# loxxous/Jampack

Hardware: AMD Instinct MI355X
Metric: MB/s compress (forward BWT + rANS encode) on 64 MiB blocks; bit-exact vs CPU ref (higher is better)
Workload: dtype u8/int32; 1 GPU; enwik8-like 100000000 B per GPU as 64 MiB blocks (2 blocks), forward BWT + rANS encode, inputs resident in HBM

## Files before the change

### jampack_amd/csrc/ans_enc.hip

```cpp
#include <vector>

#include "ans_enc.hpp"
#include "chain_pool.hpp"

using namespace jpk;
using namespace jpk_enc;

namespace {

void enc_layout(Arena &a, const EncDims &d, EncBufs &b, int what, size_t sym_total = 0, size_t lane_total = 0)
{
    const size_t tiles = (size_t)d.nch * d.tpc;
    const size_t stride = d.chunk;
    const size_t nsym = sym_total ? sym_total : (size_t)d.nch * stride;
    const size_t nlane = lane_total ? lane_total : (size_t)d.nch * 4 * rans_lane_stride(stride);
    const EncBufs keep = b;
    if (what & LAY_RANK) memset(&b, 0, sizeof b); else b = keep;
    if (what & LAY_RANK) {
        b.tilecnt = a.get<uint32_t>(tiles * 256);
        b.lastpos = a.get<int32_t>(tiles * 256);
        b.freq = a.get<int32_t>((size_t)d.nch * 256);
        b.bstart = a.get<uint32_t>((size_t)d.nch * 256);
        b.ranks = a.get<uint8_t>((size_t)d.nch * stride + 64);
    }
    if (what & LAY_RLE) {
        b.lz = a.get<uint32_t>(tiles);
        b.ext = a.get<uint32_t>(tiles);
        b.tcount = a.get<uint32_t>(tiles);
        b.toff = a.get<uint32_t>(tiles);
        b.rlen = a.get<uint32_t>(d.nch + 1);
        b.rle = a.get<uint16_t>((size_t)d.nch * stride + 64);
    }
    if (what & LAY_MODEL) {
        b.dens = a.get<uint32_t>(d.nch + 64);
        b.cmap = a.get<uint32_t>(d.nch + 64);
        b.clscnt = a.get<uint32_t>(tiles * 8);
        b.clstotal = a.get<uint32_t>((size_t)d.nch * 8);
        b.ord = a.get<uint32_t>(nsym);
        b.qhist = a.get<uint32_t>((size_t)d.nch * 6 * NQ * QSTRIDE);
        b.qcdf = a.get<uint32_t>((size_t)d.nch * 6 * NQ * QSTRIDE);
        b.exph = a.get<uint16_t>(7 * nsym);
        b.mantad = a.get<uint32_t>(nsym);
        b.cls8 = a.get<uint8_t>(nsym + 64);
        b.clist = a.get<uint32_t>(2 * ((nsym + 3) & ~(size_t)3) + 64);
        const size_t segs = (size_t)d.nch * 9 * d.tpc;
        b.seg_flag = a.get<uint32_t>(segs);
        b.seg_lo = a.get<int32_t>(segs);
        b.seg_end = a.get<int32_t>(segs);
        b.seg_start = a.get<int32_t>(segs);
        b.seg_tab = a.get<uint16_t>(segs * 32);
        b.seg_miss = a.get<uint16_t>(segs);
        b.seg_reach = a.get<uint16_t>(segs);
        b.recs = a.get<uint4>(nlane + RANS_SLACK) + (a.planning ? 0 : RANS_SLACK);
        b.pairs = (what & LAY_PLAIN) ? a.get<uint32_t>((size_t)d.nch * stride * 2) : nullptr;
    }
    if (what & LAY_RANS) {
        b.x16 = a.get<uint16_t>(nlane + 64);
        b.emask = a.get<uint32_t>(nlane / 16 + 64);
        b.etsum = a.get<uint32_t>((size_t)d.nch * emit_tiles_per_chunk(stride));
        b.fstate = a.get<uint32_t>((size_t)d.nch * 4);
        b.csize = a.get<uint32_t>(d.nch);
        b.stamp = a.get<uint64_t>(2 * (size_t)d.nch);
        b.hdr = a.get<uint8_t>((size_t)d.nch * HDR_MAX);
        b.hsize = a.get<uint32_t>(d.nch);
        b.outoff = a.get<uint64_t>(d.nch + 1);
    }
}

EncDims make_dims(uint32_t len, uint32_t chunk)
{
    EncDims d;
    d.len = len;
    d.chunk = chunk;
    d.nch = (len + chunk - 1) / chunk;
    d.tpc = (chunk + ATILE - 1) / ATILE;
    d.ncl = d.nch;
    d.cmap = nullptr;
    d.clen = nullptr;
    d.cblk = nullptr;
    d.bout = nullptr;
    d.sbase = nullptr;
    d.lbase = nullptr;
    return d;
}

__global__ __launch_bounds__(TB) void k_density(const uint8_t *__restrict__ in, EncDims d, uint32_t *__restrict__ dens)
{
    const uint32_t c = blockIdx.y, ts = blockIdx.x * ATILE * 4;
    const uint32_t clen = chunk_len(d, c);
    if (ts >= clen) return;
    const uint32_t te = (ts + ATILE * 4 < clen) ? ts + ATILE * 4 : clen;
    const uint8_t *src = in + (size_t)c * d.chunk;
    uint32_t n = 0;
    for (uint32_t i = ts + threadIdx.x * 16; i < te; i += TB * 16) {
        uint8_t prev = i ? src[i - 1] : 0;
        for (uint32_t k = 0; k < 16 && i + k < te; k++) { uint8_t v = src[i + k]; n += (v != prev); prev = v; }
    }
    n = wave_sum(n);
    if (lane_id() == 0 && n) atomicAdd(&dens[c], n);
}

__global__ __launch_bounds__(256) void k_order(EncDims d, const uint32_t *__restrict__ dens, uint32_t *__restrict__ cmap)
{
    for (uint32_t c = threadIdx.x; c < d.nch; c += blockDim.x) {
        const uint32_t v = dens[c];
        uint32_t r = 0;
        for (uint32_t k = 0; k < d.nch; k++) {
            const uint32_t w = dens[k];
            r += (w > v || (w == v && k < c)) ? 1u : 0u;
        }
        cmap[r] = c;
    }
}

constexpr uint32_t ENC_PLAN_SYM_256 = 141;

size_t enc_plan_bytes(const EncDims &d, int nblk, uint32_t sym_per_byte_256)
{
    EncBufs b;
    jpk_ctx dummy;
    Arena plan(&dummy, true);
    enc_layout(plan, d, b, LAY_RANK | LAY_RLE);
    plan.get<uint32_t>((size_t)d.nch + 1);
    plan.get<uint32_t>((size_t)d.nch + 1);
    if (nblk) { plan.get<uint32_t>(d.nch); plan.get<uint32_t>(d.nch); plan.get<uint8_t *>((size_t)nblk); }
    const size_t worst = (size_t)d.nch * d.chunk;
    size_t sym = worst / 256 * sym_per_byte_256 + 256 * (size_t)d.nch;
    if (sym > worst) sym = worst;
    enc_layout(plan, d, b, LAY_MODEL | LAY_RANS, sym, 2 * sym + 4 * 384 * (size_t)d.nch);
    return plan.need;
}

struct GroupTabs { const uint32_t *clen, *cblk; uint8_t *const *bout; int nblk; };

__global__ void k_sym_layout(EncDims d, const uint32_t *__restrict__ rlen, uint32_t *__restrict__ sbase, uint32_t *__restrict__ lbase, uint32_t *__restrict__ mail)
// ... 52 lines not shown

int enc_launch_groups(jpk_ctx *ctx, int inflight_n, uint32_t nch)
{
    int ngroups = jpk_enc_groups_for(inflight_n, nch);
    static const long groups_env = jpk_env_long("JPK_ENC_GROUPS", 0);
    if (groups_env >= 1 && groups_env <= jpk_ctx::ENC_GROUPS && (uint32_t)groups_env <= nch) ngroups = groups_env;
    for (int g = 0; g + 1 < ngroups; g++)
        if (!ctx->aux[g] && hipStreamCreateWithFlags(&ctx->aux[g], hipStreamNonBlocking) != hipSuccess) { ctx->aux[g] = nullptr; ngroups = g + 1; break; }
    return ngroups;
}

int enc_graded_groups(jpk_ctx *ctx, const uint8_t *d_in, const EncDims &d, EncBufs &b, int ngroups)
{
    hipStream_t st = ctx->stream;
    JPK_HIP(hipMemsetAsync(b.dens, 0, (size_t)d.nch * 4, st));
    JPK_LAUNCH(ctx, PROF_ENC_HIST, d.len, k_density, dim3((d.chunk + ATILE * 4 - 1) / (ATILE * 4), d.nch), dim3(TB), d_in, d, b.dens);
    JPK_LAUNCH(ctx, PROF_ENC_HIST, 0, k_order, dim3(1), dim3(256), d, b.dens, b.cmap);
    JPK_HIP(hipEventRecord(ctx->ev_pre[0], st));
    uint32_t gsz[jpk_ctx::ENC_GROUPS];
    {
        uint32_t left = d.nch;
        for (int g = 0; g < ngroups; g++) {
            uint32_t n = (g + 1 == ngroups) ? left : d.nch >> (ngroups - g);
            if (n < 2) n = 2;
            if (n > left) n = left;
            gsz[g] = n;
            left -= n;
        }
    }
    uint32_t off = 0;
    int rc = JPK_OK;
    for (int g = 0; g < ngroups && rc == JPK_OK; g++) {
        const uint32_t n = gsz[g];
        if (n == 0) continue;
        EncDims gd = d;
        gd.ncl = n; gd.cmap = b.cmap + off;
        off += n;
        hipStream_t gs = (g + 1 < ngroups) ? ctx->aux[g] : st;
        if (gs != st && hipStreamWaitEvent(gs, ctx->ev_pre[0], 0) != hipSuccess) { rc = JPK_E_DEVICE; break; }
        ctx->stream = gs;
        rc = run_model(ctx, b.rle, b.rlen, gd, b);
        if (rc == JPK_OK) rc = run_pairs(ctx, b.rle, b.rlen, gd, b);
        if (rc == JPK_OK) rc = run_chain(ctx, gd, b);
        if (rc == JPK_OK) rc = run_emit_counts(ctx, gd, b);
        ctx->stream = st;
        if (rc == JPK_OK && gs != st && hipEventRecord(ctx->ev_done[g], gs) != hipSuccess) rc = JPK_E_DEVICE;
    }
    for (int g = 0; g + 1 < ngroups && rc == JPK_OK; g++)
        if (hipStreamWaitEvent(st, ctx->ev_done[g], 0) != hipSuccess) rc = JPK_E_DEVICE;
    if (rc != JPK_OK) {
        for (int g = 0; g + 1 < jpk_ctx::ENC_GROUPS; g++) if (ctx->aux[g]) (void)hipStreamSynchronize(ctx->aux[g]);
        (void)hipStreamSynchronize(st);
    }
    return rc;
}

int enc_single_group(jpk_ctx *ctx, const EncDims &d, EncBufs &b)
{
    hipStream_t st = ctx->stream;
    JPK_TRY(run_model(ctx, b.rle, b.rlen, d, b));
    JPK_TRY(run_pairs(ctx, b.rle, b.rlen, d, b));
    JpkChainLease lease(ctx);
    if (lease.held()) {
        JPK_HIP(hipEventRecord(ctx->ev_pre[0], st));
        JPK_HIP(hipEventSynchronize(ctx->ev_pre[0]));
        ctx->stream = lease.stream;
        const int rc = run_chain(ctx, d, b);
        ctx->stream = st;
        JPK_TRY(rc);
        JPK_HIP(hipGetLastError());
        JPK_HIP(hipEventRecord(ctx->ev_done[0], lease.stream));
        JPK_HIP(hipEventSynchronize(ctx->ev_done[0]));
        lease.done();
    } else {
        JPK_TRY(run_chain(ctx, d, b));
    }
    JPK_TRY(run_emit_counts(ctx, d, b));
    return JPK_OK;
}

int encode_core(jpk_ctx *ctx, const uint8_t *d_in, EncDims &d, EncBufs &b, int inflight_n, const GroupTabs *gt = nullptr)
{
    JPK_TRY(enc_front(ctx, d_in, d, b, gt));
    JPK_HIP(hipMemsetAsync(b.qhist, 0, (size_t)d.nch * 6 * NQ * QSTRIDE * 4, ctx->stream));
    const int ngroups = enc_launch_groups(ctx, inflight_n, d.nch);
    if (ngroups >= 2) JPK_TRY(enc_graded_groups(ctx, d_in, d, b, ngroups));
    else JPK_TRY(enc_single_group(ctx, d, b));
    return run_offsets(ctx, d, b);
}
}

size_t jpk_ans_encode_arena_bytes(uint32_t len)
{
    if (len == 0) return 0;
    const EncDims d = make_dims(len, ANS_CHUNK);
    return enc_plan_bytes(d, 0, ENC_PLAN_SYM_256);
}
size_t jpk_ans_encode_arena_bytes_worst(uint32_t len)
{
    if (len == 0) return 0;
    const EncDims d = make_dims(len, ANS_CHUNK);
    return enc_plan_bytes(d, 0, 256);
}

int jpk_ans_encode_device(jpk_ctx *ctx, const uint8_t *d_in, int32_t len, uint8_t *d_out, int32_t out_cap, int32_t *out_len)
{
    const JpkCompressInflight inflight(ctx->device);
    *out_len = 0;
    ctx->stats.ans_chunks = 0;
    ctx->stats.ans_rle_symbols = 0;
    if (len == 0) return JPK_OK;
    hipStream_t st = ctx->stream;
    EncDims d = make_dims((uint32_t)len, ANS_CHUNK);
    EncBufs b;
    memset(&b, 0, sizeof b);
    JPK_TRY(encode_core(ctx, d_in, d, b, inflight.n));
    uint32_t mail[MAIL_OFFSETS_WORDS];
    JPK_TRY(jpk_read_mail(ctx, mail, MAIL_OFFSETS_WORDS));
    ctx->stats.enc_chain_cycles = (int64_t)mail_u64(mail, MAIL_CHAIN_CYCLES);
    ctx->stats.enc_chain_ns = (int64_t)mail_u64(mail, MAIL_CHAIN_TICKS) * 10;
    ctx->stats.enc_chain_steps = ((int64_t)mail[MAIL_CHAIN_RLEN] * 2 + 3) / 4;
    const uint64_t total = mail_u64(mail, MAIL_TOTAL);
    ctx->stats.ans_chunks = d.nch;
    ctx->stats.ans_rle_symbols = (int64_t)mail_u64(mail, MAIL_RLE_SYMBOLS);
    if (ctx->prof_on) {
        const uint64_t rs = (uint64_t)ctx->stats.ans_rle_symbols;
        ctx->prof_units[PROF_ENC_CLASS] += rs;
        ctx->prof_units[PROF_ENC_ADAPTIVE] += rs;
        ctx->prof_units[PROF_ENC_PAIRS] += rs;
        ctx->prof_units[PROF_ENC_RANS] += 2 * rs;
        ctx->prof_units[PROF_ENC_EMIT] += 2 * rs;
    }
    if (total > (uint64_t)out_cap) return JPK_E_CAPACITY;
    JPK_TRY(run_put(ctx, d, b, d_out));
    JPK_HIP(hipStreamSynchronize(st));
    *out_len = (int32_t)total;
    return JPK_OK;
}

size_t jpk_ans_encode_group_arena_bytes(uint32_t nchunks, int nblk)
{
    const EncDims d = make_dims(nchunks * ANS_CHUNK, ANS_CHUNK);
    return enc_plan_bytes(d, nblk, ENC_PLAN_SYM_256);
}

int jpk_ans_encode_group_device(jpk_ctx *ctx, int nblk, const uint8_t *d_stage, const uint32_t *first_chunk, const int32_t *mid_len, uint8_t *const *d_out,
                                const int32_t *out_cap, int32_t *out_len, int32_t *status)
{
    const JpkCompressInflight inflight(ctx->device);
    hipStream_t st = ctx->stream;
    std::vector<uint32_t> clen, cblk;
    for (int b = 0; b < nblk; b++) {
        out_len[b] = 0;
        status[b] = JPK_OK;
        const uint32_t ml = (uint32_t)mid_len[b], nc = (ml + ANS_CHUNK - 1) / ANS_CHUNK;
        if (clen.size() != first_chunk[b]) return JPK_E_ARG;
        for (uint32_t k = 0; k < nc; k++) {
            clen.push_back(k + 1 < nc ? (uint32_t)ANS_CHUNK : ml - k * (uint32_t)ANS_CHUNK);
            cblk.push_back((uint32_t)b);
        }
    }
    const uint32_t nch = (uint32_t)clen.size();
    if (nch == 0) return JPK_OK;
    EncDims d = make_dims(nch * ANS_CHUNK, ANS_CHUNK);
    EncBufs b;
    memset(&b, 0, sizeof b);
    const GroupTabs gt = {clen.data(), cblk.data(), d_out, nblk};
    JPK_TRY(encode_core(ctx, d_stage, d, b, inflight.n, &gt));
    uint8_t **d_bout = const_cast<uint8_t **>(d.bout);
    std::vector<uint32_t> hs(nch), cs(nch);
    JPK_HIP(hipMemcpyAsync(hs.data(), b.hsize, sizeof(uint32_t) * nch, hipMemcpyDeviceToHost, st));
    JPK_HIP(hipMemcpyAsync(cs.data(), b.csize, sizeof(uint32_t) * nch, hipMemcpyDeviceToHost, st));
    JPK_HIP(hipStreamSynchronize(st));
    std::vector<uint64_t> tot((size_t)nblk, 0);
    for (uint32_t c = 0; c < nch; c++) tot[cblk[c]] += (uint64_t)hs[c] + cs[c];
    bool all_fit = true;
    for (int k = 0; k < nblk; k++)
        if (tot[k] > (uint64_t)out_cap[k]) { status[k] = JPK_E_CAPACITY; all_fit = false; }
    if (!all_fit) {
        std::vector<uint8_t *> outs(d_out, d_out + nblk);
        for (int k = 0; k < nblk; k++) if (status[k] != JPK_OK) outs[k] = nullptr;
        JPK_HIP(hipMemcpyAsync(d_bout, outs.data(), sizeof(uint8_t *) * (size_t)nblk, hipMemcpyHostToDevice, st));
        JPK_HIP(hipStreamSynchronize(st));
    }
    JPK_TRY(run_put(ctx, d, b, nullptr));
    JPK_HIP(hipStreamSynchronize(st));
    for (int k = 0; k < nblk; k++) if (status[k] == JPK_OK) out_len[k] = (int32_t)tot[k];
    ctx->stats.ans_chunks = (int32_t)nch;
    return JPK_OK;
}

int jpk_rank_encode_device(jpk_ctx *ctx, uint8_t *d_t, int32_t *d_freq, int32_t len)
{
    if (len == 0) {
        JPK_HIP(hipMemsetAsync(d_freq, 0, 256 * 4, ctx->stream));
        return JPK_OK;
    }
    const EncDims d = make_dims((uint32_t)len, (uint32_t)len);
    EncBufs b;
    Arena plan(ctx, true);
    enc_layout(plan, d, b, LAY_RANK);
    JPK_TRY(jpk_arena_ensure(ctx, plan.need));
    Arena real(ctx, false);
    enc_layout(real, d, b, LAY_RANK);
    JPK_TRY(run_rank(ctx, d_t, d, b));
    JPK_HIP(hipMemcpyAsync(d_t, b.ranks, (size_t)len, hipMemcpyDeviceToDevice, ctx->stream));
    JPK_HIP(hipMemcpyAsync(d_freq, b.freq, 256 * 4, hipMemcpyDeviceToDevice, ctx->stream));
    return JPK_OK;
}

int jpk_rle_encode_device(jpk_ctx *ctx, const uint8_t *d_ranks, int32_t len, uint16_t *d_rle, int32_t *rlen)
{
    *rlen = 0;
    if (len == 0) return JPK_OK;
    const EncDims d = make_dims((uint32_t)len, (uint32_t)len);
    EncBufs b;
    Arena plan(ctx, true);
    enc_layout(plan, d, b, LAY_RLE);
    JPK_TRY(jpk_arena_ensure(ctx, plan.need));
    Arena real(ctx, false);
    enc_layout(real, d, b, LAY_RLE);
    JPK_TRY(run_rle(ctx, d_ranks, d, b));
    JPK_HIP(hipMemcpyAsync(ctx->d_mail->read, b.rlen, 4, hipMemcpyDeviceToDevice, ctx->stream));
    uint32_t n = 0;
    JPK_TRY(jpk_read_mail(ctx, &n, 1));
    JPK_HIP(hipMemcpyAsync(d_rle, b.rle, (size_t)n * 2, hipMemcpyDeviceToDevice, ctx->stream));
    JPK_HIP(hipStreamSynchronize(ctx->stream));
    *rlen = (int32_t)n;
    return JPK_OK;
}

int jpk_model_pairs_device(jpk_ctx *ctx, const uint16_t *d_rle, int32_t rlen, uint32_t *d_pairs)
{
    if (rlen == 0) return JPK_OK;
    const EncDims d = make_dims((uint32_t)rlen, (uint32_t)rlen);
    EncBufs b;
    Arena plan(ctx, true);
    enc_layout(plan, d, b, LAY_RLE | LAY_MODEL | LAY_PLAIN);
    JPK_TRY(jpk_arena_ensure(ctx, plan.need));
    Arena real(ctx, false);
    enc_layout(real, d, b, LAY_RLE | LAY_MODEL | LAY_PLAIN);
    uint32_t n = (uint32_t)rlen;
    JPK_HIP(hipMemcpyAsync(b.rlen, &n, 4, hipMemcpyHostToDevice, ctx->stream));
    JPK_HIP(hipStreamSynchronize(ctx->stream));
    JPK_HIP(hipMemsetAsync(b.qhist, 0, (size_t)d.nch * 6 * NQ * QSTRIDE * 4, ctx->stream));
    JPK_TRY(run_model(ctx, d_rle, b.rlen, d, b));
    JPK_TRY(run_pairs(ctx, d_rle, b.rlen, d, b));
    JPK_HIP(hipMemcpyAsync(d_pairs, b.pairs, (size_t)rlen * 8, hipMemcpyDeviceToDevice, ctx->stream));
    JPK_HIP(hipStreamSynchronize(ctx->stream));
    return JPK_OK;
}
```

### jampack_amd/csrc/ans_enc.hpp

```cpp
#pragma once
#include "ans_common.hpp"
#include "common.hpp"

namespace jpk_enc {
using namespace jpk;

constexpr int TB = 256;

struct EncDims {
    uint32_t len;
    uint32_t chunk;
    uint32_t nch;
    uint32_t tpc;
    uint32_t ncl;
    const uint32_t *cmap;
    const uint32_t *clen;
    const uint32_t *cblk;
    uint8_t *const *bout;
    const uint32_t *sbase;
    const uint32_t *lbase;
};
__device__ __forceinline__ uint32_t chunk_of(const EncDims &d, uint32_t i) { return d.cmap ? d.cmap[i] : i; }
__device__ __forceinline__ size_t sym_stride(const EncDims &d, uint32_t c, size_t rle_stride) { return d.sbase ? (size_t)(d.sbase[c + 1] - d.sbase[c]) : rle_stride; }
__device__ __forceinline__ size_t sym_base(const EncDims &d, uint32_t c, size_t rle_stride) { return d.sbase ? (size_t)d.sbase[c] : (size_t)c * rle_stride; }
__device__ __forceinline__ uint32_t chunk_len(const EncDims &d, uint32_t c)
{
    if (d.clen) return d.clen[c];
    uint64_t beg = (uint64_t)c * d.chunk;
    uint64_t left = d.len - beg;
    return left < d.chunk ? (uint32_t)left : d.chunk;
}

__host__ __device__ __forceinline__ size_t rans_lane_stride(size_t rle_stride) { return (rle_stride / 2 + 384) & ~(size_t)127; }
__device__ __forceinline__ size_t lane_stride_of(const EncDims &d, uint32_t c, size_t rle_stride) { return rans_lane_stride(sym_stride(d, c, rle_stride)); }
__device__ __forceinline__ size_t lane_base(const EncDims &d, uint32_t c, size_t rle_stride) { return d.lbase ? (size_t)d.lbase[c] : (size_t)c * 4 * rans_lane_stride(rle_stride); }

constexpr int RANS_RING = 16;
constexpr int RANS_SLACK = 16 * RANS_RING;
constexpr int ETILE = 4096;
constexpr int HDR_MAX = 259 * 5 + 1;
inline uint32_t emit_tiles_per_chunk(size_t stride) { return (uint32_t)((2 * stride + ETILE - 1) / ETILE); }

struct EncBufs {
    uint32_t *tilecnt; int32_t *lastpos; int32_t *freq; uint32_t *bstart; uint8_t *ranks;
    uint32_t *lz, *ext, *tcount, *toff, *rlen;
    uint16_t *rle;
    uint32_t *clscnt, *clstotal, *ord, *qhist, *qcdf, *dens, *cmap;
    uint8_t *cls8; uint32_t *clist;
    uint32_t *seg_flag; int32_t *seg_lo, *seg_end, *seg_start; uint16_t *seg_tab, *seg_miss, *seg_reach;
    uint16_t *exph; uint32_t *mantad, *pairs; uint4 *recs;
    uint16_t *x16; uint32_t *emask, *etsum, *fstate, *csize;
    uint64_t *stamp;
    uint8_t *hdr; uint32_t *hsize; uint64_t *outoff;
};

enum { LAY_RANK = 1, LAY_RLE = 2, LAY_MODEL = 4, LAY_RANS = 8, LAY_PLAIN = 16 };

constexpr int MAIL_TOTAL = 0;
constexpr int MAIL_RLE_SYMBOLS = 2;
constexpr int MAIL_CHAIN_CYCLES = 4;
constexpr int MAIL_CHAIN_TICKS = 6;
constexpr int MAIL_CHAIN_RLEN = 8;
constexpr int MAIL_SYM_TOTAL = 12;
constexpr int MAIL_LANE_TOTAL = 13;
constexpr int MAIL_OFFSETS_WORDS = 9, MAIL_LAYOUT_WORDS = 14;
static_assert(MAIL_LANE_TOTAL < JpkMail::READ_WORDS && MAIL_SYM_TOTAL < JpkMail::READ_WORDS, "the highest word lies inside JpkMail::read");
static_assert(MAIL_CHAIN_RLEN < MAIL_OFFSETS_WORDS && MAIL_CHAIN_TICKS + 1 < MAIL_OFFSETS_WORDS, "jpk_ans_encode_device's read covers k_out_offsets' words");
static_assert(MAIL_SYM_TOTAL < MAIL_LAYOUT_WORDS && MAIL_LANE_TOTAL < MAIL_LAYOUT_WORDS && MAIL_LAYOUT_WORDS <= JpkMail::READ_WORDS, "the front's read covers k_sym_layout's words");
static_assert(MAIL_SYM_TOTAL >= MAIL_OFFSETS_WORDS && MAIL_LANE_TOTAL >= MAIL_OFFSETS_WORDS && MAIL_SYM_TOTAL != MAIL_LANE_TOTAL, "k_sym_layout's words are none of k_out_offsets' nine");
static_assert(MAIL_TOTAL + 2 == MAIL_RLE_SYMBOLS && MAIL_RLE_SYMBOLS + 2 == MAIL_CHAIN_CYCLES && MAIL_CHAIN_CYCLES + 2 == MAIL_CHAIN_TICKS &&
              MAIL_CHAIN_TICKS + 2 == MAIL_CHAIN_RLEN, "four lo / hi pairs and one word, back to back");

int run_rank(jpk_ctx *ctx, const uint8_t *d_in, const EncDims &d, EncBufs &b);
int run_rle(jpk_ctx *ctx, const uint8_t *d_ranks, const EncDims &d, EncBufs &b);
int run_model(jpk_ctx *ctx, const uint16_t *d_rle, const uint32_t *d_rlen, const EncDims &d, EncBufs &b);
int run_pairs(jpk_ctx *ctx, const uint16_t *d_rle, const uint32_t *d_rlen, const EncDims &d, EncBufs &b);
int run_chain(jpk_ctx *ctx, const EncDims &d, EncBufs &b);
int run_emit_counts(jpk_ctx *ctx, const EncDims &d, EncBufs &b);
int run_offsets(jpk_ctx *ctx, const EncDims &d, EncBufs &b);
int run_put(jpk_ctx *ctx, const EncDims &d, EncBufs &b, uint8_t *d_out);

}
```

### jampack_amd/csrc/ans_enc_model.hip

```cpp
#include "ans_enc.hpp"

using namespace jpk;
using namespace jpk_enc;

namespace {

__global__ __launch_bounds__(TB) void k_cls_count(const uint16_t *__restrict__ rle, size_t rle_stride, EncDims d, const uint32_t *__restrict__ rlen,
                                                 uint32_t *__restrict__ clscnt)
{
    const uint32_t c = chunk_of(d, blockIdx.y), t = blockIdx.x;
    const uint32_t n = rlen[c], ts = t * ATILE;
    if (ts >= n) return;
    __shared__ uint32_t h[8];
    if (threadIdx.x < 8) h[threadIdx.x] = 0;
    __syncthreads();
    const uint16_t *src = rle + (size_t)c * rle_stride;
    uint32_t loc[8] = {0, 0, 0, 0, 0, 0, 0, 0};
    uint16_t sv[ATILE / TB];
#pragma unroll
    for (int it = 0; it < ATILE / TB; it++) {
        const uint32_t i = ts + it * TB + threadIdx.x;
        sv[it] = src[i < n ? i : n - 1];
    }
#pragma unroll
// ... 77 lines not shown
    }
    __syncthreads();
#pragma unroll
    for (int it = 0; it < IT; it++) {
        uint32_t i = ts + w * (64 * IT) + it * 64 + l;
        if (i < n) {
            uint32_t s = sy[it];
            int e = sym_class(s);
            uint32_t k = cnt[w][e] + rk[it];
            ord[sb + i] = k;
            cls8[sb + i] = (uint8_t)(e | ((s & 1u) << 3));
            if (e < 2) clist[2 * sb + (size_t)e * ((cs + 3) & ~(size_t)3) + k] = i | ((s & 1u) << 31);
            else {
                const int q = qinterval(k);
                const uint32_t m = s - (uint32_t)class_base(e);
                if (q == q0[e]) atomicAdd(&lh[e - 2][m], 1u);
                else atomicAdd(&qhist[(((size_t)c * 6 + (e - 2)) * NQ + q) * QSTRIDE + m], 1u);
            }
        }
    }
    __syncthreads();
    for (int i = threadIdx.x; i < 6 * QSTRIDE; i += TB) {
        const uint32_t v = (&lh[0][0])[i];
        if (v) {
            const int e2 = i / QSTRIDE, m = i % QSTRIDE;
            atomicAdd(&qhist[(((size_t)c * 6 + e2) * NQ + q0[e2 + 2]) * QSTRIDE + m], v);
        }
    }
}

__global__ __launch_bounds__(64) void k_quasi_build(EncDims d, const uint32_t *__restrict__ clstotal, const uint32_t *__restrict__ qhist,
                                                   uint32_t *__restrict__ qcdf)
{
    const int r = blockIdx.x, e = blockIdx.y + 2;
    const uint32_t c = chunk_of(d, blockIdx.z);
    const int A = class_alpha(e), l = lane_id();
    uint32_t *cdf = qcdf + (((size_t)c * 6 + (e - 2)) * NQ + r) * QSTRIDE;
    if (r == 0) {
        for (int i = l; i <= A; i += 64) cdf[i] = uniform_cdf(A, i);
        return;
    }
    if (clstotal[(size_t)c * 8 + e] < qbound(r)) return;
    const uint32_t *h = qhist + (((size_t)c * 6 + (e - 2)) * NQ + (r - 1)) * QSTRIDE;
    uint32_t F[3];
    uint32_t tot = 0;
#pragma unroll
    for (int k = 0; k < 3; k++) {
        int i = l + 64 * k;
        F[k] = (i < A) ? 16u * h[i] : 0u;
        tot += F[k];
    }
    tot = wave_sum(tot);
    int lg = 0;
    while ((tot >> lg) + (uint32_t)A > 65536u) lg++;
    uint32_t t2 = 0;
#pragma unroll
    for (int k = 0; k < 3; k++) {
        int i = l + 64 * k;
        F[k] = (i < A) ? (F[k] >> lg) + 1u : 0u;
        t2 += F[k];
    }
    t2 = wave_sum(t2);
    uint32_t t3 = 0;
#pragma unroll
    for (int k = 0; k < 3; k++) {
        F[k] = (65536u * F[k]) / t2;
        t3 += F[k];
    }
    t3 = wave_sum(t3);
    if (l == 0) F[0] += 65536u - t3;
    uint32_t carry = 0;
#pragma unroll
    for (int k = 0; k < 3; k++) {
        int i = l + 64 * k;
        uint32_t inc = wave_incl_sum(F[k]);
        if (i < A) cdf[i] = carry + inc - F[k];
        carry += __shfl(inc, 63, 64);
    }
    if (l == 0) cdf[A] = 65536u;
}

constexpr uint32_t AD_WARM_DEFAULT = 320;
static_assert(AD_WARM_DEFAULT % 64 == 0 && AD_WARM_DEFAULT >= 320 && AD_WARM_DEFAULT <= 4096, "whole waves of warm-up items, guarantee above");

struct AdRec {
    bool exp;
    int i;
    int cls;
    int A;
    __device__ __forceinline__ AdRec(uint32_t rec) : exp(rec < 7), i(rec < 7 ? (int)rec + 1 : 1), cls((int)rec - 7), A(rec < 7 ? 8 : 2) {}
    __device__ __forceinline__ int32_t init() const { return (int32_t)uniform_cdf(A, i); }
    __device__ __forceinline__ int32_t smin() const { return i; }
    __device__ __forceinline__ int32_t smax() const { return i + 65536 - A; }
};

__host__ __device__ __forceinline__ size_t clist_stride(size_t rle_stride) { return (rle_stride + 3) & ~(size_t)3; }

struct AdStream {
    const uint8_t *c8;
    const uint32_t *list;
    uint32_t n;
};
__device__ __forceinline__ AdStream ad_stream(const EncDims &d, const AdRec &r, uint32_t c, const uint8_t *cls8, const uint32_t *clist, size_t rle_stride,
                                              const uint32_t *rlen, const uint32_t *clstotal)
{
    AdStream st;
    const size_t sb = sym_base(d, c, rle_stride), cs = sym_stride(d, c, rle_stride);
    st.c8 = cls8 + sb;
    st.list = r.exp ? nullptr : clist + 2 * sb + (size_t)r.cls * clist_stride(cs);
    st.n = r.exp ? rlen[c] : clstotal[(size_t)c * 8 + r.cls];
    return st;
}

template <class F>
__device__ __forceinline__ void ad_for_each(const AdRec &r, const AdStream &st, uint32_t t0, uint32_t t1, F f)
{
    uint32_t t = t0;
    if (r.exp) {
        const uint8_t *p = st.c8;
        while (t < t1 && (t & 15u)) { f(t, (int)(p[t] & 7u)); t++; }
        if (t + 64 <= t1) {
            uint4 v[4];
#pragma unroll
            for (int q = 0; q < 4; q++) v[q] = *reinterpret_cast<const uint4 *>(p + t + 16 * q);
            for (; t + 64 <= t1; t += 64) {
                const uint32_t tn = (t + 128 <= t1) ? t + 64 : t;
                uint4 nv[4];
#pragma unroll
                for (int q = 0; q < 4; q++) nv[q] = *reinterpret_cast<const uint4 *>(p + tn + 16 * q);
#pragma unroll
                for (int q = 0; q < 4; q++) {
                    const uint32_t w[4] = {v[q].x, v[q].y, v[q].z, v[q].w};
#pragma unroll
                    for (int k = 0; k < 16; k++) f(t + 16 * q + k, (int)((w[k >> 2] >> (8 * (k & 3))) & 7u));
                }
#pragma unroll
                for (int q = 0; q < 4; q++) v[q] = nv[q];
            }
        }
        if (t + 16 <= t1) {
            uint4 v = *reinterpret_cast<const uint4 *>(p + t);
            for (; t + 16 <= t1; t += 16) {
                const uint32_t tn = (t + 32 <= t1) ? t + 16 : t;
                const uint4 nv = *reinterpret_cast<const uint4 *>(p + tn);
                const uint32_t w[4] = {v.x, v.y, v.z, v.w};
#pragma unroll
                for (int k = 0; k < 16; k++) f(t + k, (int)((w[k >> 2] >> (8 * (k & 3))) & 7u));
                v = nv;
            }
        }
        while (t < t1) { f(t, (int)(p[t] & 7u)); t++; }
    } else {
        const uint32_t *p = st.list;
        while (t < t1 && (t & 3u)) { const uint32_t e = p[t]; f(e & 0x7FFFFFFFu, (int)(e >> 31)); t++; }
        if (t + 16 <= t1) {
            uint4 v[4];
#pragma unroll
            for (int q = 0; q < 4; q++) v[q] = *reinterpret_cast<const uint4 *>(p + t + 4 * q);
            for (; t + 16 <= t1; t += 16) {
                const uint32_t tn = (t + 32 <= t1) ? t + 16 : t;
                uint4 nv[4];
#pragma unroll
                for (int q = 0; q < 4; q++) nv[q] = *reinterpret_cast<const uint4 *>(p + tn + 4 * q);
#pragma unroll
                for (int q = 0; q < 4; q++) {
                    f(v[q].x & 0x7FFFFFFFu, (int)(v[q].x >> 31));
// ... 13 lines not shown
                f(v.x & 0x7FFFFFFFu, (int)(v.x >> 31));
                f(v.y & 0x7FFFFFFFu, (int)(v.y >> 31));
                f(v.z & 0x7FFFFFFFu, (int)(v.z >> 31));
                f(v.w & 0x7FFFFFFFu, (int)(v.w >> 31));
                v = nv;
            }
        }
        while (t < t1) { const uint32_t e = p[t]; f(e & 0x7FFFFFFFu, (int)(e >> 31)); t++; }
    }
}

__device__ __forceinline__ int32_t ad_run_write(const AdRec &r, const AdStream &st, uint32_t t0, uint32_t t1, int32_t x,
                                                uint16_t *__restrict__ hist, uint32_t *__restrict__ ma)
{
    if (r.exp) {
        const int i = r.i;
        const uint8_t *p = st.c8;
        uint32_t t = t0;
        while (t < t1 && (t & 15u)) { hist[t] = (uint16_t)x; x = adapt_step(x, i, (int)(p[t] & 7u), 8); t++; }
        if (t + 64 <= t1) {
            uint4 v[4];
#pragma unroll
            for (int q = 0; q < 4; q++) v[q] = *reinterpret_cast<const uint4 *>(p + t + 16 * q);
            for (; t + 64 <= t1; t += 64) {
                const uint32_t tn = (t + 128 <= t1) ? t + 64 : t;
                uint4 nv[4];
#pragma unroll
                for (int q = 0; q < 4; q++) nv[q] = *reinterpret_cast<const uint4 *>(p + tn + 16 * q);
#pragma unroll
                for (int q = 0; q < 4; q++) {
                    const uint32_t w[4] = {v[q].x, v[q].y, v[q].z, v[q].w};
                    uint32_t o[8];
#pragma unroll
                    for (int k = 0; k < 16; k++) {
                        if (k & 1) o[k >> 1] |= (uint32_t)x << 16;
                        else o[k >> 1] = (uint32_t)x & 0xffffu;
                        x = adapt_step(x, i, (int)((w[k >> 2] >> (8 * (k & 3))) & 7u), 8);
                    }
                    uint4 *qq = reinterpret_cast<uint4 *>(hist + t + 16 * q);
                    qq[0] = make_uint4(o[0], o[1], o[2], o[3]);
                    qq[1] = make_uint4(o[4], o[5], o[6], o[7]);
                }
#pragma unroll
                for (int q = 0; q < 4; q++) v[q] = nv[q];
            }
        }
        if (t + 16 <= t1) {
            uint4 v = *reinterpret_cast<const uint4 *>(p + t);
            for (; t + 16 <= t1; t += 16) {
                const uint32_t tn = (t + 32 <= t1) ? t + 16 : t;
                const uint4 nv = *reinterpret_cast<const uint4 *>(p + tn);
                const uint32_t w[4] = {v.x, v.y, v.z, v.w};
                uint32_t o[8];
#pragma unroll
                for (int k = 0; k < 16; k++) {
                    if (k & 1) o[k >> 1] |= (uint32_t)x << 16;
                    else o[k >> 1] = (uint32_t)x & 0xffffu;
                    x = adapt_step(x, i, (int)((w[k >> 2] >> (8 * (k & 3))) & 7u), 8);
                }
                uint4 *q = reinterpret_cast<uint4 *>(hist + t);
                q[0] = make_uint4(o[0], o[1], o[2], o[3]);
                q[1] = make_uint4(o[4], o[5], o[6], o[7]);
                v = nv;
            }
        }
        while (t < t1) { hist[t] = (uint16_t)x; x = adapt_step(x, i, (int)(p[t] & 7u), 8); t++; }
    } else {
        ad_for_each(r, st, t0, t1, [&](uint32_t t, int m) {
            const uint32_t l0 = m ? (uint32_t)x : 0u, fr = m ? 65536u - (uint32_t)x : (uint32_t)x;
            ma[t] = l0 | (fr << 16);
            x = adapt_step(x, 1, m, 2);
        });
    }
    return x;
}

struct AdArgs {
    const uint8_t *cls8; const uint32_t *clist; size_t rle_stride; const uint32_t *rlen; const uint32_t *clstotal;
    const uint32_t *clsbase;
    uint16_t *exph; uint32_t *mantad;
    uint32_t warm;
    uint32_t *seg_flag; int32_t *seg_lo, *seg_end, *seg_start; uint16_t *seg_tab;
    uint16_t *seg_miss, *seg_reach;
};

__global__ __launch_bounds__(64) void k_adapt_a(EncDims d, AdArgs a)
{
    const uint32_t c = chunk_of(d, blockIdx.z), rec = blockIdx.y;
    const uint32_t k = blockIdx.x * 64 + threadIdx.x;
    const AdRec r(rec);
    const AdStream st = ad_stream(d, r, c, a.cls8, a.clist, a.rle_stride, a.rlen, a.clstotal);
    const uint32_t nt = (st.n + ATILE - 1) / ATILE;
    const bool valid = k < nt;
    const uint32_t t0 = valid ? k * ATILE : 0u, t1 = !valid ? 0u : (t0 + ATILE < st.n) ? t0 + ATILE : st.n;
    const uint32_t len = t1 - t0;
    const int i = r.i, A = r.A;
    int32_t lo = r.init(), hi = lo;
    if (valid && k != 0) {
        lo = r.smin(); hi = r.smax();
        ad_for_each(r, st, t0 - a.warm, t0, [&](uint32_t, int sy) { lo = adapt_step(lo, i, sy, A); hi = adapt_step(hi, i, sy, A); });
    }
    const size_t so = ((size_t)c * 9 + rec) * d.tpc + k;
    const int32_t lo0 = lo, hi0 = hi;
    const bool plat = valid && r.exp && lo != hi && hi == r.smax() && lo == r.smax() - 31;
    bool ident = false;
    if (plat) {
        const uint32_t *cb = a.clsbase + ((size_t)c * d.tpc + k) * 8;
        uint32_t reach = 0;
        for (int e = r.i; e < 8; e++) reach += ((k + 1 < nt) ? cb[8 + e] : a.clstotal[(size_t)c * 8 + e]) - cb[e];
        ident = reach == 0;
    }
    const bool walk = valid && !ident;
    bool open = walk && lo != hi, quiet = plat;
    uint32_t miss = 0, fr = 0, u = 0;
    uint16_t *hist = a.exph + 7 * sym_base(d, c, a.rle_stride) + (size_t)(rec < 7 ? rec : 0) * sym_stride(d, c, a.rle_stride);
    uint32_t *ma = a.mantad + sym_base(d, c, a.rle_stride);
    if (r.exp) {
        const uint8_t *p = st.c8 + t0;
        const int32_t top = r.smax();
        uint4 v[4];
        if (__ballot(open && 64u <= len)) {
#pragma unroll
            for (int q = 0; q < 4; q++) v[q] = *reinterpret_cast<const uint4 *>(p + ((walk && 64u <= len) ? 16 * q : 0));
        }
        while (__ballot(open && u + 64 <= len)) {
            const bool in = walk && u + 64 <= len;
            const uint32_t un = (in && u + 128 <= len) ? u + 64 : (in ? u : 0u);
            uint4 nv[4];
#pragma unroll
            for (int q = 0; q < 4; q++) nv[q] = *reinterpret_cast<const uint4 *>(p + un + 16 * q);
            if (in) {
#pragma unroll
                for (int q = 0; q < 4; q++) {
                    const uint32_t w[4] = {v[q].x, v[q].y, v[q].z, v[q].w};
                    const bool one = lo == hi;
                    uint32_t o[8];
#pragma unroll
                    for (int j = 0; j < 16; j++) {
                        if (j & 1) o[j >> 1] |= (uint32_t)lo << 16;
                        else o[j >> 1] = (uint32_t)lo & 0xffffu;
                        const int sy = (int)((w[j >> 2] >> (8 * (j & 3))) & 7u);
                        lo = adapt_step(lo, i, sy, 8);
                        hi = adapt_step(hi, i, sy, 8);
                    }
                    if (one) {
                        uint4 *qq = reinterpret_cast<uint4 *>(hist + t0 + u + 16 * q);
                        qq[0] = make_uint4(o[0], o[1], o[2], o[3]);
                        qq[1] = make_uint4(o[4], o[5], o[6], o[7]);
                    }
                    if (quiet) { if (hi == top) fr = u + 16 * q + 16; else quiet = false; }
                    if (open && lo == hi) { open = false; miss = u + 16 * q + 16; }
                }
            }
#pragma unroll
            for (int q = 0; q < 4; q++) v[q] = nv[q];
            u += 64;
        }
        if (walk && u > (len & ~63u)) u = len & ~63u;
    } else {
        const uint32_t *p = st.list + t0;
        uint4 v[4];
        if (__ballot(open && 16u <= len)) {
#pragma unroll
            for (int q = 0; q < 4; q++) v[q] = *reinterpret_cast<const uint4 *>(p + ((walk && 16u <= len) ? 4 * q : 0));
        }
        while (__ballot(open && u + 16 <= len)) {
            const bool in = walk && u + 16 <= len;
            const uint32_t un = (in && u + 32 <= len) ? u + 16 : (in ? u : 0u);
            uint4 nv[4];
#pragma unroll
            for (int q = 0; q < 4; q++) nv[q] = *reinterpret_cast<const uint4 *>(p + un + 4 * q);
            if (in) {
                const bool one = lo == hi;
#pragma unroll
                for (int q = 0; q < 4; q++) {
                    const uint32_t w[4] = {v[q].x, v[q].y, v[q].z, v[q].w};
#pragma unroll
                    for (int j = 0; j < 4; j++) {
                        const int m = (int)(w[j] >> 31);
                        if (one) {
                            const uint32_t l0 = m ? (uint32_t)lo : 0u, f = m ? 65536u - (uint32_t)lo : (uint32_t)lo;
                            ma[w[j] & 0x7FFFFFFFu] = l0 | (f << 16);
                        }
                        lo = adapt_step(lo, 1, m, 2);
                        hi = adapt_step(hi, 1, m, 2);
                    }
                }
                if (open && lo == hi) { open = false; miss = u + 16; }
            }
#pragma unroll
            for (int q = 0; q < 4; q++) v[q] = nv[q];
            u += 16;
        }
        if (walk && u > (len & ~15u)) u = len & ~15u;
    }
    if (!valid) return;
    if (ident) {
        a.seg_flag[so] = 2u;
        return;
    }
    if (open) {
        ad_for_each(r, st, t0 + u, t1, [&](uint32_t, int sy) { lo = adapt_step(lo, i, sy, A); hi = adapt_step(hi, i, sy, A); });
        a.seg_miss[so] = (uint16_t)len;
        a.seg_reach[so] = (uint16_t)fr;
        if (lo == hi) { a.seg_flag[so] = 3u; a.seg_end[so] = lo; }
        else { a.seg_flag[so] = 0u; a.seg_lo[so] = lo0; a.seg_end[so] = hi0; }
        return;
    }
    a.seg_flag[so] = miss ? 3u : 1u;
    a.seg_miss[so] = (uint16_t)miss;
    a.seg_reach[so] = (uint16_t)fr;
    a.seg_end[so] = ad_run_write(r, st, t0 + u, t1, lo, hist, ma);
}

__global__ __launch_bounds__(64) void k_adapt_tab(EncDims d, AdArgs a)
{
    const uint32_t c = chunk_of(d, blockIdx.z), rec = blockIdx.y;
    const uint32_t k = blockIdx.x * 2 + (threadIdx.x >> 5);
    const int q = threadIdx.x & 31;
    const AdRec r(rec);
    const AdStream st = ad_stream(d, r, c, a.cls8, a.clist, a.rle_stride, a.rlen, a.clstotal);
    const uint32_t nt = (st.n + ATILE - 1) / ATILE;
    if (k >= nt) return;
    const size_t so = ((size_t)c * 9 + rec) * d.tpc + k;
    if (a.seg_flag[so]) return;
    const uint32_t t0 = k * ATILE, t1 = (t0 + ATILE < st.n) ? t0 + ATILE : st.n;
    const int32_t lo = a.seg_lo[so], hi = a.seg_end[so];
    int32_t x = (lo + q < hi) ? lo + q : hi;
    const int i = r.i, A = r.A;
    ad_for_each(r, st, t0, t1, [&](uint32_t, int sy) { x = adapt_step(x, i, sy, A); });
    a.seg_tab[so * 32 + q] = (uint16_t)(x - 1);
}

__global__ __launch_bounds__(64) void k_adapt_b(EncDims d, AdArgs a)
{
    const uint32_t g = blockIdx.x * 64 + threadIdx.x;
    const uint32_t rec = g & 15u;
    if ((g >> 4) >= d.ncl || rec >= 9) return;
    const uint32_t c = chunk_of(d, g >> 4);
    const AdRec r(rec);
    const AdStream st = ad_stream(d, r, c, a.cls8, a.clist, a.rle_stride, a.rlen, a.clstotal);
    const uint32_t nt = (st.n + ATILE - 1) / ATILE;
    int32_t x = r.init();
    for (uint32_t k = 0; k < nt; k++) {
        const size_t so = ((size_t)c * 9 + rec) * d.tpc + k;
        const uint32_t flag = a.seg_flag[so];
        if (flag == 1u) x = a.seg_end[so];
        else if (flag == 2u) a.seg_start[so] = x;
        else if (flag == 3u) { a.seg_start[so] = x; x = a.seg_end[so]; }
        else {
            a.seg_start[so] = x;
            int q = x - a.seg_lo[so];
            q = q < 0 ? 0 : (q > 31 ? 31 : q);
            x = (int32_t)a.seg_tab[so * 32 + q] + 1;
        }
    }
}

__global__ __launch_bounds__(64) void k_adapt_c(EncDims d, AdArgs a)
{
    const uint32_t c = chunk_of(d, blockIdx.z), rec = blockIdx.y;
    const uint32_t k = blockIdx.x * 64 + threadIdx.x;
    const AdRec r(rec);
    const AdStream st = ad_stream(d, r, c, a.cls8, a.clist, a.rle_stride, a.rlen, a.clstotal);
    const uint32_t nt = (st.n + ATILE - 1) / ATILE;
    if (k >= nt) return;
    const size_t so = ((size_t)c * 9 + rec) * d.tpc + k;
    const uint32_t flag = a.seg_flag[so];
    if (flag == 1u) return;
    const uint32_t t0 = k * ATILE, t1 = (t0 + ATILE < st.n) ? t0 + ATILE : st.n;
    const uint32_t miss = flag == 2u ? t1 - t0 : a.seg_miss[so], fr = flag == 2u ? t1 - t0 : a.seg_reach[so];
    uint16_t *hist = a.exph + 7 * sym_base(d, c, a.rle_stride) + (size_t)(rec < 7 ? rec : 0) * sym_stride(d, c, a.rle_stride);
    const int32_t x0 = a.seg_start[so];
    if (fr) {
        const uint32_t x = (uint32_t)x0 & 0xffffu, xx = x | (x << 16);
        uint32_t t = t0;
        for (; t + 8 <= t0 + fr; t += 8) *reinterpret_cast<uint4 *>(hist + t) = make_uint4(xx, xx, xx, xx);
        for (; t < t0 + fr; t++) hist[t] = (uint16_t)x;
    }
    if (fr < miss) ad_run_write(r, st, t0 + fr, t0 + miss, x0, hist, a.mantad + sym_base(d, c, a.rle_stride));
}

}

namespace jpk_enc {

int run_model(jpk_ctx *ctx, const uint16_t *d_rle, const uint32_t *d_rlen, const EncDims &d, EncBufs &b)
{
    const size_t stride = d.chunk;
    JPK_LAUNCH(ctx, PROF_ENC_CLASS, 0, k_cls_count, dim3(d.tpc, d.ncl), dim3(TB), d_rle, stride, d, d_rlen, b.clscnt);
    JPK_LAUNCH(ctx, PROF_ENC_CLASS, 0, k_cls_prefix, dim3(jpk_grid((size_t)d.ncl * 8, 64)), dim3(64), d, d_rlen, b.clscnt, b.clstotal);
    JPK_LAUNCH(ctx, PROF_ENC_CLASS, 0, k_cls_ord, dim3(d.tpc, d.ncl), dim3(TB), d_rle, stride, d, d_rlen, b.clscnt, b.ord, b.qhist, b.cls8, b.clist);
    JPK_LAUNCH(ctx, PROF_ENC_CLASS, 0, k_quasi_build, dim3(NQ, 6, d.ncl), dim3(64), d, b.clstotal, b.qhist, b.qcdf);
    AdArgs aa;
    aa.cls8 = b.cls8; aa.clist = b.clist; aa.rle_stride = stride; aa.rlen = d_rlen; aa.clstotal = b.clstotal; aa.clsbase = b.clscnt;
    aa.exph = b.exph; aa.mantad = b.mantad;
    aa.warm = AD_WARM_DEFAULT;
    aa.seg_flag = b.seg_flag; aa.seg_lo = b.seg_lo; aa.seg_end = b.seg_end; aa.seg_start = b.seg_start; aa.seg_tab = b.seg_tab;
    aa.seg_miss = b.seg_miss; aa.seg_reach = b.seg_reach;
    JPK_LAUNCH(ctx, PROF_ENC_ADAPTIVE, 0, k_adapt_a, dim3((d.tpc + 63) / 64, 9, d.ncl), dim3(64), d, aa);
    JPK_LAUNCH(ctx, PROF_ENC_ADAPTIVE, 0, k_adapt_tab, dim3((d.tpc + 1) / 2, 9, d.ncl), dim3(64), d, aa);
    JPK_LAUNCH(ctx, PROF_ENC_ADAPTIVE, 0, k_adapt_b, dim3(jpk_grid((size_t)d.ncl * 16, 64)), dim3(64), d, aa);
    JPK_LAUNCH(ctx, PROF_ENC_ADAPTIVE, 0, k_adapt_c, dim3((d.tpc + 63) / 64, 9, d.ncl), dim3(64), d, aa);
    JPK_HIP(hipGetLastError());
    return JPK_OK;
}

}
```

Before: 6344 MB/s.

## Split adaptive-model segments into sub-tiles with compacted table worklist and wave scan

Adaptive-model segments shrink from a full tile to AD_SUB-sized sub-tiles, so the per-segment walk in k_adapt_a/k_adapt_c exposes more parallelism. Segments that need a 32-entry transfer table are compacted into a worklist via an atomic counter, so k_adapt_tab runs a fixed grid over only real work instead of a dense grid. k_adapt_b replaces a serial per-thread chain walk with a wave-level ballot/shuffle scan over 64 segments at a time. The cost is more segment metadata, a repeated warm-up per sub-tile, an atomic counter per chunk, and a counter word appended to the zeroed qhist region.

```diff
diff --git a/jampack_amd/csrc/ans_enc.hip b/jampack_amd/csrc/ans_enc.hip
--- a/jampack_amd/csrc/ans_enc.hip
+++ b/jampack_amd/csrc/ans_enc.hip
@@ -37,13 +37,14 @@
         b.clscnt = a.get<uint32_t>(tiles * 8);
         b.clstotal = a.get<uint32_t>((size_t)d.nch * 8);
         b.ord = a.get<uint32_t>(nsym);
-        b.qhist = a.get<uint32_t>((size_t)d.nch * 6 * NQ * QSTRIDE);
+        b.qhist = a.get<uint32_t>(model_zero_words(d.nch));
+        b.seg_nwork = a.planning ? nullptr : b.qhist + (size_t)d.nch * 6 * NQ * QSTRIDE;
         b.qcdf = a.get<uint32_t>((size_t)d.nch * 6 * NQ * QSTRIDE);
         b.exph = a.get<uint16_t>(7 * nsym);
         b.mantad = a.get<uint32_t>(nsym);
         b.cls8 = a.get<uint8_t>(nsym + 64);
         b.clist = a.get<uint32_t>(2 * ((nsym + 3) & ~(size_t)3) + 64);
-        const size_t segs = (size_t)d.nch * 9 * d.tpc;
+        const size_t segs = (size_t)d.nch * 9 * d.tpc * AD_PER_TILE;
         b.seg_flag = a.get<uint32_t>(segs);
         b.seg_lo = a.get<int32_t>(segs);
         b.seg_end = a.get<int32_t>(segs);
@@ -51,6 +52,7 @@
         b.seg_tab = a.get<uint16_t>(segs * 32);
         b.seg_miss = a.get<uint16_t>(segs);
         b.seg_reach = a.get<uint16_t>(segs);
+        b.seg_work = a.get<uint32_t>(segs);
         b.recs = a.get<uint4>(nlane + RANS_SLACK) + (a.planning ? 0 : RANS_SLACK);
         b.pairs = (what & LAY_PLAIN) ? a.get<uint32_t>((size_t)d.nch * stride * 2) : nullptr;
     }
@@ -269,7 +271,7 @@
 int encode_core(jpk_ctx *ctx, const uint8_t *d_in, EncDims &d, EncBufs &b, int inflight_n, const GroupTabs *gt = nullptr)
 {
     JPK_TRY(enc_front(ctx, d_in, d, b, gt));
-    JPK_HIP(hipMemsetAsync(b.qhist, 0, (size_t)d.nch * 6 * NQ * QSTRIDE * 4, ctx->stream));
+    JPK_HIP(hipMemsetAsync(b.qhist, 0, model_zero_words(d.nch) * 4, ctx->stream));
     const int ngroups = enc_launch_groups(ctx, inflight_n, d.nch);
     if (ngroups >= 2) JPK_TRY(enc_graded_groups(ctx, d_in, d, b, ngroups));
     else JPK_TRY(enc_single_group(ctx, d, b));
@@ -430,7 +432,7 @@
     uint32_t n = (uint32_t)rlen;
     JPK_HIP(hipMemcpyAsync(b.rlen, &n, 4, hipMemcpyHostToDevice, ctx->stream));
     JPK_HIP(hipStreamSynchronize(ctx->stream));
-    JPK_HIP(hipMemsetAsync(b.qhist, 0, (size_t)d.nch * 6 * NQ * QSTRIDE * 4, ctx->stream));
+    JPK_HIP(hipMemsetAsync(b.qhist, 0, model_zero_words(d.nch) * 4, ctx->stream));
     JPK_TRY(run_model(ctx, d_rle, b.rlen, d, b));
     JPK_TRY(run_pairs(ctx, d_rle, b.rlen, d, b));
     JPK_HIP(hipMemcpyAsync(d_pairs, b.pairs, (size_t)rlen * 8, hipMemcpyDeviceToDevice, ctx->stream));
diff --git a/jampack_amd/csrc/ans_enc.hpp b/jampack_amd/csrc/ans_enc.hpp
--- a/jampack_amd/csrc/ans_enc.hpp
+++ b/jampack_amd/csrc/ans_enc.hpp
@@ -41,6 +41,14 @@
 constexpr int HDR_MAX = 259 * 5 + 1;
 inline uint32_t emit_tiles_per_chunk(size_t stride) { return (uint32_t)((2 * stride + ETILE - 1) / ETILE); }
 
+#ifndef JPK_AD_SUB
+#define JPK_AD_SUB 1024
+#endif
+constexpr int AD_SUB = JPK_AD_SUB;
+constexpr int AD_PER_TILE = ATILE / AD_SUB;
+static_assert(AD_SUB >= 512 && AD_SUB <= ATILE && (AD_SUB & (AD_SUB - 1)) == 0 && ATILE % AD_SUB == 0, "a power of two that divides the tile, longer than a warm-up");
+inline size_t model_zero_words(uint32_t nch) { return (size_t)nch * 6 * NQ * QSTRIDE + nch; }
+
 struct EncBufs {
     uint32_t *tilecnt; int32_t *lastpos; int32_t *freq; uint32_t *bstart; uint8_t *ranks;
     uint32_t *lz, *ext, *tcount, *toff, *rlen;
@@ -48,6 +56,7 @@
     uint32_t *clscnt, *clstotal, *ord, *qhist, *qcdf, *dens, *cmap;
     uint8_t *cls8; uint32_t *clist;
     uint32_t *seg_flag; int32_t *seg_lo, *seg_end, *seg_start; uint16_t *seg_tab, *seg_miss, *seg_reach;
+    uint32_t *seg_work, *seg_nwork;
     uint16_t *exph; uint32_t *mantad, *pairs; uint4 *recs;
     uint16_t *x16; uint32_t *emask, *etsum, *fstate, *csize;
     uint64_t *stamp;
diff --git a/jampack_amd/csrc/ans_enc_model.hip b/jampack_amd/csrc/ans_enc_model.hip
--- a/jampack_amd/csrc/ans_enc_model.hip
+++ b/jampack_amd/csrc/ans_enc_model.hip
@@ -183,6 +183,7 @@
 
 constexpr uint32_t AD_WARM_DEFAULT = 320;
 static_assert(AD_WARM_DEFAULT % 64 == 0 && AD_WARM_DEFAULT >= 320 && AD_WARM_DEFAULT <= 4096, "whole waves of warm-up items, guarantee above");
+static_assert(AD_WARM_DEFAULT <= (uint32_t)AD_SUB && AD_SUB % 64 == 0, "a warm-up starts inside the stream; whole 64-item groups, 16-byte stores");
 
 struct AdRec {
     bool exp;
@@ -362,7 +363,10 @@
     uint32_t warm;
     uint32_t *seg_flag; int32_t *seg_lo, *seg_end, *seg_start; uint16_t *seg_tab;
     uint16_t *seg_miss, *seg_reach;
+    uint32_t *work, *nwork;
+    uint32_t spc;
 };
+__device__ __forceinline__ uint32_t ad_subs(const AdStream &st) { return (st.n + AD_SUB - 1) / AD_SUB; }
 
 __global__ __launch_bounds__(64) void k_adapt_a(EncDims d, AdArgs a)
 {
@@ -370,9 +374,10 @@
     const uint32_t k = blockIdx.x * 64 + threadIdx.x;
     const AdRec r(rec);
     const AdStream st = ad_stream(d, r, c, a.cls8, a.clist, a.rle_stride, a.rlen, a.clstotal);
-    const uint32_t nt = (st.n + ATILE - 1) / ATILE;
-    const bool valid = k < nt;
-    const uint32_t t0 = valid ? k * ATILE : 0u, t1 = !valid ? 0u : (t0 + ATILE < st.n) ? t0 + ATILE : st.n;
+    const uint32_t ns = ad_subs(st);
+    if (blockIdx.x * 64 >= ns) return;
+    const bool valid = k < ns;
+    const uint32_t t0 = valid ? k * AD_SUB : 0u, t1 = !valid ? 0u : (t0 + AD_SUB < st.n) ? t0 + AD_SUB : st.n;
     const uint32_t len = t1 - t0;
     const int i = r.i, A = r.A;
     int32_t lo = r.init(), hi = lo;
@@ -380,14 +385,15 @@
         lo = r.smin(); hi = r.smax();
         ad_for_each(r, st, t0 - a.warm, t0, [&](uint32_t, int sy) { lo = adapt_step(lo, i, sy, A); hi = adapt_step(hi, i, sy, A); });
     }
-    const size_t so = ((size_t)c * 9 + rec) * d.tpc + k;
+    const size_t so = ((size_t)c * 9 + rec) * a.spc + k;
     const int32_t lo0 = lo, hi0 = hi;
     const bool plat = valid && r.exp && lo != hi && hi == r.smax() && lo == r.smax() - 31;
     bool ident = false;
     if (plat) {
-        const uint32_t *cb = a.clsbase + ((size_t)c * d.tpc + k) * 8;
+        const uint32_t tile = k / AD_PER_TILE, nt = (st.n + ATILE - 1) / ATILE;
+        const uint32_t *cb = a.clsbase + ((size_t)c * d.tpc + tile) * 8;
         uint32_t reach = 0;
-        for (int e = r.i; e < 8; e++) reach += ((k + 1 < nt) ? cb[8 + e] : a.clstotal[(size_t)c * 8 + e]) - cb[e];
+        for (int e = r.i; e < 8; e++) reach += ((tile + 1 < nt) ? cb[8 + e] : a.clstotal[(size_t)c * 8 + e]) - cb[e];
         ident = reach == 0;
     }
     const bool walk = valid && !ident;
@@ -481,10 +487,17 @@
     }
     if (open) {
         ad_for_each(r, st, t0 + u, t1, [&](uint32_t, int sy) { lo = adapt_step(lo, i, sy, A); hi = adapt_step(hi, i, sy, A); });
+        if (plat && hi == r.smax()) {
+            a.seg_flag[so] = 2u;
+            return;
+        }
         a.seg_miss[so] = (uint16_t)len;
         a.seg_reach[so] = (uint16_t)fr;
         if (lo == hi) { a.seg_flag[so] = 3u; a.seg_end[so] = lo; }
-        else { a.seg_flag[so] = 0u; a.seg_lo[so] = lo0; a.seg_end[so] = hi0; }
+        else {
+            a.seg_flag[so] = 0u; a.seg_lo[so] = lo0; a.seg_end[so] = hi0;
+            a.work[atomicAdd(a.nwork, 1u)] = (uint32_t)so;
+        }
         return;
     }
     a.seg_flag[so] = miss ? 3u : 1u;
@@ -493,47 +506,69 @@
     a.seg_end[so] = ad_run_write(r, st, t0 + u, t1, lo, hist, ma);
 }
 
+constexpr uint32_t AD_TAB_BLOCKS = 128;
 __global__ __launch_bounds__(64) void k_adapt_tab(EncDims d, AdArgs a)
 {
-    const uint32_t c = chunk_of(d, blockIdx.z), rec = blockIdx.y;
-    const uint32_t k = blockIdx.x * 2 + (threadIdx.x >> 5);
+    const uint32_t n = *a.nwork;
     const int q = threadIdx.x & 31;
+    for (uint32_t w = blockIdx.x * 2 + (threadIdx.x >> 5); w < n; w += gridDim.x * 2) {
+        const uint32_t so = a.work[w];
+        const uint32_t k = so % a.spc, rec = (so / a.spc) % 9u, c = so / a.spc / 9u;
+        const AdRec r(rec);
+        const AdStream st = ad_stream(d, r, c, a.cls8, a.clist, a.rle_stride, a.rlen, a.clstotal);
+        const uint32_t t0 = k * AD_SUB, t1 = (t0 + AD_SUB < st.n) ? t0 + AD_SUB : st.n;
+        const int32_t lo = a.seg_lo[so], hi = a.seg_end[so];
+        int32_t x = (lo + q < hi) ? lo + q : hi;
+        const int i = r.i, A = r.A;
+        ad_for_each(r, st, t0, t1, [&](uint32_t, int sy) { x = adapt_step(x, i, sy, A); });
+        a.seg_tab[(size_t)so * 32 + q] = (uint16_t)(x - 1);
+    }
+}
+
+__global__ __launch_bounds__(64) void k_adapt_b(EncDims d, AdArgs a)
+{
+    const uint32_t c = chunk_of(d, blockIdx.y), rec = blockIdx.x;
+    const int l = threadIdx.x;
     const AdRec r(rec);
     const AdStream st = ad_stream(d, r, c, a.cls8, a.clist, a.rle_stride, a.rlen, a.clstotal);
-    const uint32_t nt = (st.n + ATILE - 1) / ATILE;
-    if (k >= nt) return;
-    const size_t so = ((size_t)c * 9 + rec) * d.tpc + k;
-    if (a.seg_flag[so]) return;
-    const uint32_t t0 = k * ATILE, t1 = (t0 + ATILE < st.n) ? t0 + ATILE : st.n;
-    const int32_t lo = a.seg_lo[so], hi = a.seg_end[so];
-    int32_t x = (lo + q < hi) ? lo + q : hi;
-    const int i = r.i, A = r.A;
-    ad_for_each(r, st, t0, t1, [&](uint32_t, int sy) { x = adapt_step(x, i, sy, A); });
-    a.seg_tab[so * 32 + q] = (uint16_t)(x - 1);
-}
-
-__global__ __launch_bounds__(64) void k_adapt_b(EncDims d, AdArgs a)
-{
-    const uint32_t g = blockIdx.x * 64 + threadIdx.x;
-    const uint32_t rec = g & 15u;
-    if ((g >> 4) >= d.ncl || rec >= 9) return;
-    const uint32_t c = chunk_of(d, g >> 4);
-    const AdRec r(rec);
-    const AdStream st = ad_stream(d, r, c, a.cls8, a.clist, a.rle_stride, a.rlen, a.clstotal);
-    const uint32_t nt = (st.n + ATILE - 1) / ATILE;
-    int32_t x = r.init();
-    for (uint32_t k = 0; k < nt; k++) {
-        const size_t so = ((size_t)c * 9 + rec) * d.tpc + k;
-        const uint32_t flag = a.seg_flag[so];
-        if (flag == 1u) x = a.seg_end[so];
-        else if (flag == 2u) a.seg_start[so] = x;
-        else if (flag == 3u) { a.seg_start[so] = x; x = a.seg_end[so]; }
-        else {
-            a.seg_start[so] = x;
-            int q = x - a.seg_lo[so];
+    const uint32_t ns = ad_subs(st);
+    const size_t s0 = ((size_t)c * 9 + rec) * a.spc;
+    const uint64_t lt = lanemask_lt();
+    __shared__ uint4 rows[64][4];
+    int32_t carry = r.init();
+    for (uint32_t base = 0; base < ns; base += 64) {
+        const uint32_t k = base + l;
+        const bool valid = k < ns;
+        const size_t so = s0 + k;
+        const uint32_t flag = valid ? a.seg_flag[so] : 2u;
+        const bool cst = flag == 1u || flag == 3u, tab = flag == 0u;
+        int32_t out = cst ? a.seg_end[so] : 0;
+        const uint64_t cm = __ballot(cst), tm = __ballot(tab);
+        int32_t tlo = 0;
+        if (tm) {
+            if (tab) {
+                tlo = a.seg_lo[so];
+                const uint4 *row = reinterpret_cast<const uint4 *>(a.seg_tab + so * 32);
+#pragma unroll
+                for (int j = 0; j < 4; j++) rows[l][j] = row[j];
+            }
+            __syncthreads();
+        }
+        const uint64_t below = (cm | tm) & lt;
+        const int src = below ? 63 - __clzll((long long)below) : -1;
+        int32_t in = __shfl(out, src < 0 ? 0 : src, 64);
+        if (src < 0) in = carry;
+        for (uint64_t m = tm; m; m &= m - 1) {
+            const int tl = __ffsll((unsigned long long)m) - 1;
+            int q = __shfl(in, tl, 64) - __shfl(tlo, tl, 64);
             q = q < 0 ? 0 : (q > 31 ? 31 : q);
-            x = (int32_t)a.seg_tab[so * 32 + q] + 1;
-        }
+            const int32_t o = (int32_t)reinterpret_cast<const uint16_t *>(&rows[tl][0])[q] + 1;
+            if (l == tl) out = o;
+            if (src == tl) in = o;
+        }
+        if (tm) __syncthreads();
+        if (valid && flag != 1u) a.seg_start[so] = in;
+        carry = __shfl((cst || tab) ? out : in, 63, 64);
     }
 }
 
@@ -543,12 +578,11 @@
     const uint32_t k = blockIdx.x * 64 + threadIdx.x;
     const AdRec r(rec);
     const AdStream st = ad_stream(d, r, c, a.cls8, a.clist, a.rle_stride, a.rlen, a.clstotal);
-    const uint32_t nt = (st.n + ATILE - 1) / ATILE;
-    if (k >= nt) return;
-    const size_t so = ((size_t)c * 9 + rec) * d.tpc + k;
+    if (k >= ad_subs(st)) return;
+    const size_t so = ((size_t)c * 9 + rec) * a.spc + k;
     const uint32_t flag = a.seg_flag[so];
     if (flag == 1u) return;
-    const uint32_t t0 = k * ATILE, t1 = (t0 + ATILE < st.n) ? t0 + ATILE : st.n;
+    const uint32_t t0 = k * AD_SUB, t1 = (t0 + AD_SUB < st.n) ? t0 + AD_SUB : st.n;
     const uint32_t miss = flag == 2u ? t1 - t0 : a.seg_miss[so], fr = flag == 2u ? t1 - t0 : a.seg_reach[so];
     uint16_t *hist = a.exph + 7 * sym_base(d, c, a.rle_stride) + (size_t)(rec < 7 ? rec : 0) * sym_stride(d, c, a.rle_stride);
     const int32_t x0 = a.seg_start[so];
@@ -578,10 +612,13 @@
     aa.warm = AD_WARM_DEFAULT;
     aa.seg_flag = b.seg_flag; aa.seg_lo = b.seg_lo; aa.seg_end = b.seg_end; aa.seg_start = b.seg_start; aa.seg_tab = b.seg_tab;
     aa.seg_miss = b.seg_miss; aa.seg_reach = b.seg_reach;
-    JPK_LAUNCH(ctx, PROF_ENC_ADAPTIVE, 0, k_adapt_a, dim3((d.tpc + 63) / 64, 9, d.ncl), dim3(64), d, aa);
-    JPK_LAUNCH(ctx, PROF_ENC_ADAPTIVE, 0, k_adapt_tab, dim3((d.tpc + 1) / 2, 9, d.ncl), dim3(64), d, aa);
-    JPK_LAUNCH(ctx, PROF_ENC_ADAPTIVE, 0, k_adapt_b, dim3(jpk_grid((size_t)d.ncl * 16, 64)), dim3(64), d, aa);
-    JPK_LAUNCH(ctx, PROF_ENC_ADAPTIVE, 0, k_adapt_c, dim3((d.tpc + 63) / 64, 9, d.ncl), dim3(64), d, aa);
+    aa.spc = d.tpc * AD_PER_TILE;
+    const size_t first = d.cmap ? (size_t)(d.cmap - b.cmap) : 0;
+    aa.work = b.seg_work + first * 9 * aa.spc; aa.nwork = b.seg_nwork + first;
+    JPK_LAUNCH(ctx, PROF_ENC_ADAPTIVE, 0, k_adapt_a, dim3((aa.spc + 63) / 64, 9, d.ncl), dim3(64), d, aa);
+    JPK_LAUNCH(ctx, PROF_ENC_ADAPTIVE, 0, k_adapt_tab, dim3(AD_TAB_BLOCKS), dim3(64), d, aa);
+    JPK_LAUNCH(ctx, PROF_ENC_ADAPTIVE, 0, k_adapt_b, dim3(9, d.ncl), dim3(64), d, aa);
+    JPK_LAUNCH(ctx, PROF_ENC_ADAPTIVE, 0, k_adapt_c, dim3((aa.spc + 63) / 64, 9, d.ncl), dim3(64), d, aa);
     JPK_HIP(hipGetLastError());
     return JPK_OK;
 }
```

After: 6273 MB/s. -1.1%, worse.
